# aliabdelkader/FusionTransformer

Measured on AMD Instinct MI355X. Metric: frames/sec fwd+bwd (SemanticKITTI synth), whole job, higher is better.
Workload: dtype f32

## Files before the change

### fusiontransformer_amd/csrc/ftx_attn.hip

```cpp
#include "ftx_common.h"

using namespace ftx;

typedef float f32x16 __attribute__((ext_vector_type(16)));

constexpr int HD = 64;
constexpr int TS = 68;
constexpr float LOG2E = 1.4426950408889634f;
constexpr float LN2 = 0.6931471805599453f;

__device__ inline int acc_row(int g, int h) { return (g & 3) + 8 * (g >> 2) + 4 * h; }

__device__ inline float exp2_raw(float x) { return __builtin_amdgcn_exp2f(x); }

__device__ inline const float *qkv_row(const float *qkv, int b, int t, int which, int hd, int T, int nh) {
  return qkv + ((((int64_t)b * T + t) * 3 + which) * nh + hd) * HD;
}

__device__ inline void load_frag(const float *row, int h, bool valid, float (&f)[32]) {
#pragma unroll
  for (int t = 0; t < 8; ++t) {
    float4 v = make_float4(0.f, 0.f, 0.f, 0.f);
    if (valid) v = *(const float4 *)(row + 8 * t + 4 * h);
    f[4 * t + 0] = v.x; f[4 * t + 1] = v.y; f[4 * t + 2] = v.z; f[4 * t + 3] = v.w;
  }
}

__device__ inline void mfma_lds_x_frag(const float *lds_tile, int l31, int h, const float (&frag)[32], f32x16 &acc) {
  const float *rp = lds_tile + l31 * TS + 4 * h;
#pragma unroll
  for (int t = 0; t < 8; ++t) {
    float4 a = *(const float4 *)(rp + 8 * t);
    acc = __builtin_amdgcn_mfma_f32_32x32x2f32(a.x, frag[4 * t + 0], acc, 0, 0, 0);
    acc = __builtin_amdgcn_mfma_f32_32x32x2f32(a.y, frag[4 * t + 1], acc, 0, 0, 0);
    acc = __builtin_amdgcn_mfma_f32_32x32x2f32(a.z, frag[4 * t + 2], acc, 0, 0, 0);
    acc = __builtin_amdgcn_mfma_f32_32x32x2f32(a.w, frag[4 * t + 3], acc, 0, 0, 0);
  }
}

__device__ inline void mfma_frag_x_lds(const float (&frag)[32], const float *lds_tile, int l31, int h, f32x16 &acc) {
  const float *rp = lds_tile + l31 * TS + 4 * h;
#pragma unroll
  for (int t = 0; t < 8; ++t) {
    float4 b = *(const float4 *)(rp + 8 * t);
    acc = __builtin_amdgcn_mfma_f32_32x32x2f32(frag[4 * t + 0], b.x, acc, 0, 0, 0);
    acc = __builtin_amdgcn_mfma_f32_32x32x2f32(frag[4 * t + 1], b.y, acc, 0, 0, 0);
    acc = __builtin_amdgcn_mfma_f32_32x32x2f32(frag[4 * t + 2], b.z, acc, 0, 0, 0);
    acc = __builtin_amdgcn_mfma_f32_32x32x2f32(frag[4 * t + 3], b.w, acc, 0, 0, 0);
  }
}

__device__ inline void mfma_ldsT_x_acc(const float *lds_tile, int col_off, int l31, int h, const f32x16 &x, f32x16 &out) {
#pragma unroll
  for (int g = 0; g < 16; ++g) {
    float a = lds_tile[acc_row(g, h) * TS + col_off + l31];
    out = __builtin_amdgcn_mfma_f32_32x32x2f32(a, x[g], out, 0, 0, 0);
  }
}

template <int NT>
__device__ inline void tile_prefetch(const float *qkv, int b, int hd, int which, int t0, int T, int nh, int tid, float4 (&r)[512 / NT]) {
#pragma unroll
  for (int q = 0; q < 512 / NT; ++q) {
    int e = q * NT + tid;
    int row = e >> 4, c4 = (e & 15) * 4;
    float4 v = make_float4(0.f, 0.f, 0.f, 0.f);
    if (t0 + row < T) v = *(const float4 *)(qkv_row(qkv, b, t0 + row, which, hd, T, nh) + c4);
    r[q] = v;
  }
}
template <int NT>
__device__ inline void tile_store(float *lds_tile, int tid, const float4 (&r)[512 / NT]) {
#pragma unroll
  for (int q = 0; q < 512 / NT; ++q) {
    int e = q * NT + tid;
    int row = e >> 4, c4 = (e & 15) * 4;
    *(float4 *)&lds_tile[row * TS + c4] = r[q];
  }
}
template <int NT>
__device__ inline void tile_prefetch_o(const float *o, int b, int hd, int t0, int T, int nh, int tid, float4 (&r)[512 / NT]) {
#pragma unroll
  for (int q = 0; q < 512 / NT; ++q) {
    int e = q * NT + tid;
    int row = e >> 4, c4 = (e & 15) * 4;
    float4 v = make_float4(0.f, 0.f, 0.f, 0.f);
    if (t0 + row < T) v = *(const float4 *)(o + (((int64_t)b * T + t0 + row) * nh + hd) * HD + c4);
    r[q] = v;
  }
}

template <int QW>
__device__ inline void group_sync() {
  if (QW == 1) {
    __builtin_amdgcn_fence(__ATOMIC_RELEASE, "wavefront");
    __builtin_amdgcn_wave_barrier();
    __builtin_amdgcn_fence(__ATOMIC_ACQUIRE, "wavefront");
  } else {
    __syncthreads();
  }
}
constexpr int cmax(int a, int b) { return a > b ? a : b; }
template <int QW, int SPLIT, int NREG, int EXTRA>
constexpr int smem_floats() { return cmax(SPLIT * (2 * 32 * TS + EXTRA), cmax(SPLIT / 2, 1) * QW * NREG * 64); }

template <int QW, int SPLIT, int NTILES>
__device__ inline void merge_sum(float *smem, int grp, int wave, int lane, f32x16 (&acc)[NTILES]) {
  if (SPLIT == 1) return;
#pragma unroll
  for (int s = 1; s < SPLIT; s <<= 1) {
    float *cw = smem + ((grp / (2 * s)) * QW + wave) * (16 * NTILES) * 64 + lane;
    __syncthreads();
    if ((grp & (2 * s - 1)) == s) {
#pragma unroll
      for (int t = 0; t < NTILES; ++t)
#pragma unroll
        for (int g = 0; g < 16; ++g) cw[(t * 16 + g) * 64] = acc[t][g];
    }
    __syncthreads();
    if ((grp & (2 * s - 1)) == 0 && grp + s < SPLIT) {
#pragma unroll
      for (int t = 0; t < NTILES; ++t)
#pragma unroll
        for (int g = 0; g < 16; ++g) acc[t][g] += cw[(t * 16 + g) * 64];
    }
  }
}

template <int QW, int SPLIT>
__global__ __launch_bounds__(64 * QW * SPLIT) void attn_fwd_kernel(const float *__restrict__ qkv, int T, int nh, float scale,
                                                                   float *__restrict__ out, float *__restrict__ lse) {
  constexpr int NT = 64 * QW;
  __shared__ __attribute__((aligned(16))) float smem[smem_floats<QW, SPLIT, 34, 0>()];
  const int tid = threadIdx.x % NT, grp = threadIdx.x / NT;
  float *Ks = smem + grp * (2 * 32 * TS), *Vs = Ks + 32 * TS;
  const int wave = tid >> 6, lane = tid & 63, l31 = lane & 31, h = lane >> 5;
  const int hd = blockIdx.y, b = blockIdx.z;
  const int q = blockIdx.x * (32 * QW) + wave * 32 + l31;
  const bool qv = q < T;
  const bool wave_live = blockIdx.x * (32 * QW) + wave * 32 < T;
  const float sl2 = scale * LOG2E;

  float qf[32];
  load_frag(qkv_row(qkv, b, qv ? q : 0, 0, hd, T, nh), h, qv, qf);
#pragma unroll
  for (int i = 0; i < 32; ++i) qf[i] *= sl2;

  f32x16 o0, o1;
#pragma unroll
  for (int g = 0; g < 16; ++g) o0[g] = o1[g] = 0.f;
  float m = -INFINITY, l = 0.f;

  const int ntiles = (T + 31) / 32;
  const int iters = (ntiles + SPLIT - 1) / SPLIT;
  float4 rk[512 / NT], rv[512 / NT];
  tile_prefetch<NT>(qkv, b, hd, 1, grp * 32, T, nh, tid, rk);
  tile_prefetch<NT>(qkv, b, hd, 2, grp * 32, T, nh, tid, rv);
  for (int it = 0; it < iters; ++it) {
    const int kt = it * SPLIT + grp;
    tile_store<NT>(Ks, tid, rk);
    tile_store<NT>(Vs, tid, rv);
    group_sync<QW>();
    if (it + 1 < iters) {
      tile_prefetch<NT>(qkv, b, hd, 1, (kt + SPLIT) * 32, T, nh, tid, rk);
      tile_prefetch<NT>(qkv, b, hd, 2, (kt + SPLIT) * 32, T, nh, tid, rv);
    }
    if (kt < ntiles && wave_live) {
      f32x16 st;
#pragma unroll
      for (int g = 0; g < 16; ++g) st[g] = 0.f;
      mfma_lds_x_frag(Ks, l31, h, qf, st);
      if (kt == ntiles - 1) {
#pragma unroll
        for (int g = 0; g < 16; ++g)
          if (kt * 32 + acc_row(g, h) >= T) st[g] = -INFINITY;
      }
      float mx = fmaxf(fmaxf(fmaxf(st[0], st[1]), fmaxf(st[2], st[3])), fmaxf(fmaxf(st[4], st[5]), fmaxf(st[6], st[7])));
      mx = fmaxf(mx, fmaxf(fmaxf(fmaxf(st[8], st[9]), fmaxf(st[10], st[11])), fmaxf(fmaxf(st[12], st[13]), fmaxf(st[14], st[15]))));
      mx = fmaxf(mx, __shfl_xor(mx, 32, 64));
      const float m_new = fmaxf(m, mx);
      float rs = 0.f;
#pragma unroll
      for (int g = 0; g < 16; ++g) {
        float p = exp2_raw(st[g] - m_new);
        st[g] = p;
        rs += p;
      }
      rs += __shfl_xor(rs, 32, 64);
      if (__any(m_new != m)) {
        const float alpha = exp2_raw(m - m_new);
        l *= alpha;
#pragma unroll
        for (int g = 0; g < 16; ++g) {
          o0[g] *= alpha;
          o1[g] *= alpha;
        }
      }
      l += rs;
      m = m_new;
      mfma_ldsT_x_acc(Vs, 0, l31, h, st, o0);
      mfma_ldsT_x_acc(Vs, 32, l31, h, st, o1);
    }
    group_sync<QW>();
  }
  if (SPLIT > 1) {
#pragma unroll
    for (int s = 1; s < SPLIT; s <<= 1) {
      float *cw = smem + ((grp / (2 * s)) * QW + wave) * 34 * 64 + lane;
      __syncthreads();
      if ((grp & (2 * s - 1)) == s) {
        cw[0] = m;
        cw[64] = l;
#pragma unroll
        for (int g = 0; g < 16; ++g) {
          cw[(2 + g) * 64] = o0[g];
          cw[(18 + g) * 64] = o1[g];
        }
      }
      __syncthreads();
      if ((grp & (2 * s - 1)) == 0 && grp + s < SPLIT) {
        const float m1 = cw[0], l1 = cw[64];
        const float mt = fmaxf(m, m1);
        const float a0 = (m == -INFINITY) ? 0.f : exp2f(m - mt), a1 = (m1 == -INFINITY) ? 0.f : exp2f(m1 - mt);
        l = l * a0 + l1 * a1;
        m = mt;
#pragma unroll
        for (int g = 0; g < 16; ++g) {
          o0[g] = o0[g] * a0 + cw[(2 + g) * 64] * a1;
          o1[g] = o1[g] * a0 + cw[(18 + g) * 64] * a1;
        }
      }
    }
  }
  if (qv && grp == 0) {
    const float inv = 1.f / l;
    float *op = out + (((int64_t)b * T + q) * nh + hd) * HD;
#pragma unroll
    for (int g4 = 0; g4 < 4; ++g4) {
      int r = acc_row(4 * g4, h);
      *(float4 *)(op + r) = make_float4(o0[4 * g4] * inv, o0[4 * g4 + 1] * inv, o0[4 * g4 + 2] * inv, o0[4 * g4 + 3] * inv);
      *(float4 *)(op + 32 + r) = make_float4(o1[4 * g4] * inv, o1[4 * g4 + 1] * inv, o1[4 * g4 + 2] * inv, o1[4 * g4 + 3] * inv);
    }
    if (h == 0) lse[((int64_t)b * nh + hd) * T + q] = (m + log2f(l)) * LN2;
  }
}

__global__ void attn_delta_kernel(const float *__restrict__ o, const float *__restrict__ go, int64_t rows, int T, int nh, float *__restrict__ delta) {
  const int64_t gid = (blockIdx.x * (int64_t)blockDim.x + threadIdx.x) >> 4;
  const int sub = threadIdx.x & 15;
  if (gid >= rows) return;
  float4 a = *(const float4 *)(o + gid * HD + sub * 4);
  float4 g = *(const float4 *)(go + gid * HD + sub * 4);
  float s = a.x * g.x + a.y * g.y + a.z * g.z + a.w * g.w;
#pragma unroll
  for (int off = 8; off > 0; off >>= 1) s += __shfl_xor(s, off, 16);
  if (sub == 0) {
    int64_t bt = gid / nh;
    int hd = (int)(gid - bt * nh);
    int64_t bb = bt / T;
    int t = (int)(bt - bb * T);
    delta[(bb * nh + hd) * T + t] = s;
  }
}

template <int QW, int SPLIT>
__global__ __launch_bounds__(64 * QW * SPLIT) void attn_bwd_kv_kernel(const float *__restrict__ qkv, const float *__restrict__ go,
                                                                      const float *__restrict__ lse, const float *__restrict__ delta, int T,
                                                                      int nh, float scale, float *__restrict__ gqkv) {
  constexpr int NT = 64 * QW;
  __shared__ __attribute__((aligned(16))) float smem[smem_floats<QW, SPLIT, 64, 64>()];
  const int tid = threadIdx.x % NT, grp = threadIdx.x / NT;
  float *Qs = smem + grp * (2 * 32 * TS + 64), *Gs = Qs + 32 * TS, *s_lse = Gs + 32 * TS, *s_delta = s_lse + 32;
  const int wave = tid >> 6, lane = tid & 63, l31 = lane & 31, h = lane >> 5;
  const int hd = blockIdx.y, b = blockIdx.z;
  const int key = blockIdx.x * (32 * QW) + wave * 32 + l31;
  const bool kv = key < T;
  const bool wave_live = blockIdx.x * (32 * QW) + wave * 32 < T;
  const float sl2 = scale * LOG2E;

  float kf[32], vf[32];
  load_frag(qkv_row(qkv, b, kv ? key : 0, 1, hd, T, nh), h, kv, kf);
  load_frag(qkv_row(qkv, b, kv ? key : 0, 2, hd, T, nh), h, kv, vf);
#pragma unroll
  for (int i = 0; i < 32; ++i) kf[i] *= sl2;

  f32x16 acc[4];
#pragma unroll
  for (int t = 0; t < 4; ++t)
#pragma unroll
    for (int g = 0; g < 16; ++g) acc[t][g] = 0.f;

  const int ntiles = (T + 31) / 32;
  const int iters = (ntiles + SPLIT - 1) / SPLIT;
  float4 rq[512 / NT], rg[512 / NT];
  tile_prefetch<NT>(qkv, b, hd, 0, grp * 32, T, nh, tid, rq);
  tile_prefetch_o<NT>(go, b, hd, grp * 32, T, nh, tid, rg);
  for (int it = 0; it < iters; ++it) {
    const int qt = it * SPLIT + grp;
    tile_store<NT>(Qs, tid, rq);
    tile_store<NT>(Gs, tid, rg);
    if (tid < 32) {
      int t = qt * 32 + tid;
      s_lse[tid] = t < T ? lse[((int64_t)b * nh + hd) * T + t] * LOG2E : 0.f;
      s_delta[tid] = t < T ? delta[((int64_t)b * nh + hd) * T + t] : 0.f;
    }
    group_sync<QW>();
    if (it + 1 < iters) {
      tile_prefetch<NT>(qkv, b, hd, 0, (qt + SPLIT) * 32, T, nh, tid, rq);
      tile_prefetch_o<NT>(go, b, hd, (qt + SPLIT) * 32, T, nh, tid, rg);
    }
    if (qt < ntiles && wave_live) {
      f32x16 s, dp;
#pragma unroll
      for (int g = 0; g < 16; ++g) s[g] = dp[g] = 0.f;
      mfma_lds_x_frag(Qs, l31, h, kf, s);
      mfma_lds_x_frag(Gs, l31, h, vf, dp);
#pragma unroll
      for (int g = 0; g < 16; ++g) {
        const int r = acc_row(g, h);
        const float p = exp2_raw(s[g] - s_lse[r]);
        s[g] = p;
        dp[g] = p * (dp[g] - s_delta[r]) * scale;
      }
      if (qt == ntiles - 1) {
#pragma unroll
        for (int g = 0; g < 16; ++g)
          if (qt * 32 + acc_row(g, h) >= T) s[g] = dp[g] = 0.f;
      }
      mfma_ldsT_x_acc(Gs, 0, l31, h, s, acc[0]);
      mfma_ldsT_x_acc(Gs, 32, l31, h, s, acc[1]);
      mfma_ldsT_x_acc(Qs, 0, l31, h, dp, acc[2]);
      mfma_ldsT_x_acc(Qs, 32, l31, h, dp, acc[3]);
    }
    group_sync<QW>();
  }
  merge_sum<QW, SPLIT, 4>(smem, grp, wave, lane, acc);
  if (kv && grp == 0) {
    float *kp = gqkv + ((((int64_t)b * T + key) * 3 + 1) * nh + hd) * HD;
    float *vp = gqkv + ((((int64_t)b * T + key) * 3 + 2) * nh + hd) * HD;
#pragma unroll
    for (int g4 = 0; g4 < 4; ++g4) {
      int r = acc_row(4 * g4, h);
      *(float4 *)(vp + r) = make_float4(acc[0][4 * g4], acc[0][4 * g4 + 1], acc[0][4 * g4 + 2], acc[0][4 * g4 + 3]);
      *(float4 *)(vp + 32 + r) = make_float4(acc[1][4 * g4], acc[1][4 * g4 + 1], acc[1][4 * g4 + 2], acc[1][4 * g4 + 3]);
      *(float4 *)(kp + r) = make_float4(acc[2][4 * g4], acc[2][4 * g4 + 1], acc[2][4 * g4 + 2], acc[2][4 * g4 + 3]);
      *(float4 *)(kp + 32 + r) = make_float4(acc[3][4 * g4], acc[3][4 * g4 + 1], acc[3][4 * g4 + 2], acc[3][4 * g4 + 3]);
    }
  }
}

template <int QW, int SPLIT>
__global__ __launch_bounds__(64 * QW * SPLIT) void attn_bwd_q_kernel(const float *__restrict__ qkv, const float *__restrict__ go,
                                                                     const float *__restrict__ lse, const float *__restrict__ delta, int T,
                                                                     int nh, float scale, float *__restrict__ gqkv) {
  constexpr int NT = 64 * QW;
  __shared__ __attribute__((aligned(16))) float smem[smem_floats<QW, SPLIT, 32, 0>()];
  const int tid = threadIdx.x % NT, grp = threadIdx.x / NT;
  float *Ks = smem + grp * (2 * 32 * TS), *Vs = Ks + 32 * TS;
  const int wave = tid >> 6, lane = tid & 63, l31 = lane & 31, h = lane >> 5;
  const int hd = blockIdx.y, b = blockIdx.z;
  const int q = blockIdx.x * (32 * QW) + wave * 32 + l31;
  const bool qv = q < T;
  const bool wave_live = blockIdx.x * (32 * QW) + wave * 32 < T;
  const float sl2 = scale * LOG2E;

  float qf[32], gf[32];
  load_frag(qkv_row(qkv, b, qv ? q : 0, 0, hd, T, nh), h, qv, qf);
#pragma unroll
  for (int i = 0; i < 32; ++i) qf[i] *= sl2;
  load_frag(go + (((int64_t)b * T + (qv ? q : 0)) * nh + hd) * HD, h, qv, gf);
  const float my_lse = qv ? lse[((int64_t)b * nh + hd) * T + q] * LOG2E : 0.f;
  const float my_delta = qv ? delta[((int64_t)b * nh + hd) * T + q] : 0.f;

  f32x16 acc[2];
#pragma unroll
  for (int g = 0; g < 16; ++g) acc[0][g] = acc[1][g] = 0.f;

  const int ntiles = (T + 31) / 32;
  const int iters = (ntiles + SPLIT - 1) / SPLIT;
  float4 rk[512 / NT], rv[512 / NT];
  tile_prefetch<NT>(qkv, b, hd, 1, grp * 32, T, nh, tid, rk);
  tile_prefetch<NT>(qkv, b, hd, 2, grp * 32, T, nh, tid, rv);
  for (int it = 0; it < iters; ++it) {
    const int kt = it * SPLIT + grp;
    tile_store<NT>(Ks, tid, rk);
    tile_store<NT>(Vs, tid, rv);
    group_sync<QW>();
    if (it + 1 < iters) {
      tile_prefetch<NT>(qkv, b, hd, 1, (kt + SPLIT) * 32, T, nh, tid, rk);
      tile_prefetch<NT>(qkv, b, hd, 2, (kt + SPLIT) * 32, T, nh, tid, rv);
    }
    if (kt < ntiles && wave_live) {
      f32x16 st, dpt;
#pragma unroll
      for (int g = 0; g < 16; ++g) st[g] = dpt[g] = 0.f;
      mfma_lds_x_frag(Ks, l31, h, qf, st);
      mfma_lds_x_frag(Vs, l31, h, gf, dpt);
#pragma unroll
      for (int g = 0; g < 16; ++g) {
        const float p = exp2_raw(st[g] - my_lse);
        dpt[g] = p * (dpt[g] - my_delta) * scale;
      }
      if (kt == ntiles - 1) {
#pragma unroll
        for (int g = 0; g < 16; ++g)
          if (kt * 32 + acc_row(g, h) >= T) dpt[g] = 0.f;
      }
      mfma_ldsT_x_acc(Ks, 0, l31, h, dpt, acc[0]);
      mfma_ldsT_x_acc(Ks, 32, l31, h, dpt, acc[1]);
    }
    group_sync<QW>();
  }
  merge_sum<QW, SPLIT, 2>(smem, grp, wave, lane, acc);
  if (qv && grp == 0) {
    float *qp = gqkv + ((((int64_t)b * T + q) * 3 + 0) * nh + hd) * HD;
#pragma unroll
    for (int g4 = 0; g4 < 4; ++g4) {
      int r = acc_row(4 * g4, h);
      *(float4 *)(qp + r) = make_float4(acc[0][4 * g4], acc[0][4 * g4 + 1], acc[0][4 * g4 + 2], acc[0][4 * g4 + 3]);
      *(float4 *)(qp + 32 + r) = make_float4(acc[1][4 * g4], acc[1][4 * g4 + 1], acc[1][4 * g4 + 2], acc[1][4 * g4 + 3]);
    }
  }
}

static int attn_check(const char *who, int b, int t, int h, int d) {
  FTX_REQUIRE(b >= 1 && t >= 1 && h >= 1, "%s: bad size", who);
  FTX_REQUIRE(d == HD, "%s: head dim must be 64 (got %d)", who, d);
  FTX_REQUIRE(b <= 65535 && h <= 65535, "%s: batch / heads exceed the grid limits", who);
  return FTX_OK;
}

static bool attn_tiling_built(int qw, int split) {
  return (qw == 0 && split == 0) || (qw == 4 && split == 2) || (qw == 2 && (split == 2 || split == 4)) ||
         (qw == 1 && (split == 2 || split == 4 || split == 8));
}
static void attn_config(int b, int t, int h, bool backward, int &qw, int &split) {
  if (qw != 0) return;
  const int64_t wave_tiles = (int64_t)ceil_div(t, 32) * h * b;
  const int64_t simds = 4 * 256;
  if (wave_tiles * 4 <= simds) { qw = 1; split = backward ? 4 : 8; }
  else if (wave_tiles * 2 <= simds) { qw = 2; split = 4; }
  else { qw = 4; split = 2; }
}

#define ATTN_DISPATCH(KERNEL, ...)                                                                               \
  do {                                                                                                           \
    dim3 grid((unsigned)ceil_div(t, 32 * qw), (unsigned)h, (unsigned)b);                                         \
    if (qw == 4) KERNEL<4, 2><<<grid, 512, 0, st>>>(__VA_ARGS__);                                                \
    else if (qw == 2 && split == 2) KERNEL<2, 2><<<grid, 256, 0, st>>>(__VA_ARGS__);                             \
    else if (qw == 2) KERNEL<2, 4><<<grid, 512, 0, st>>>(__VA_ARGS__);                                           \
    else if (split == 2) KERNEL<1, 2><<<grid, 128, 0, st>>>(__VA_ARGS__);                                        \
    else if (split == 4) KERNEL<1, 4><<<grid, 256, 0, st>>>(__VA_ARGS__);                                        \
    else KERNEL<1, 8><<<grid, 512, 0, st>>>(__VA_ARGS__);                                                        \
  } while (0)

extern "C" int ftx_attn_fwd_tiled(const float *qkv, int32_t b, int32_t t, int32_t h, int32_t d, float scale, float *out, float *lse, int32_t qw,
                                  int32_t split, void *stream) {
  int rc = attn_check("ftx_attn_fwd", b, t, h, d);
  if (rc != FTX_OK) return rc;
  FTX_REQUIRE(qkv && out && lse, "ftx_attn_fwd: null pointer");
  FTX_REQUIRE(attn_tiling_built(qw, split), "ftx_attn_fwd_tiled: (%d, %d) is not a built tiling", qw, split);
  hipStream_t st = (hipStream_t)stream;
  attn_config(b, t, h, false, qw, split);
  ATTN_DISPATCH(attn_fwd_kernel, qkv, t, h, scale, out, lse);
  return check_launch("ftx_attn_fwd");
}

extern "C" int ftx_attn_fwd(const float *qkv, int32_t b, int32_t t, int32_t h, int32_t d, float scale, float *out, float *lse, void *stream) {
  return ftx_attn_fwd_tiled(qkv, b, t, h, d, scale, out, lse, 0, 0, stream);
}

extern "C" size_t ftx_attn_bwd_workspace_bytes(int32_t b, int32_t t, int32_t h) {
  if (b <= 0 || t <= 0 || h <= 0) return 256;
  return sizeof(float) * (size_t)b * t * h + 256;
}

extern "C" int ftx_attn_bwd_tiled(const float *qkv, const float *out, const float *grad_out, const float *lse, int32_t b, int32_t t, int32_t h,
                                  int32_t d, float scale, float *grad_qkv, void *workspace, size_t workspace_bytes, int32_t qw, int32_t split,
                                  void *stream) {
  int rc = attn_check("ftx_attn_bwd", b, t, h, d);
  if (rc != FTX_OK) return rc;
  FTX_REQUIRE(qkv && out && grad_out && lse && grad_qkv && workspace, "ftx_attn_bwd: null pointer");
  FTX_REQUIRE(attn_tiling_built(qw, split), "ftx_attn_bwd_tiled: (%d, %d) is not a built tiling", qw, split);
  if (workspace_bytes < ftx_attn_bwd_workspace_bytes(b, t, h)) {
    set_error("ftx_attn_bwd: workspace %zu < required %zu", workspace_bytes, ftx_attn_bwd_workspace_bytes(b, t, h));
    return FTX_EWORKSPACE;
  }
  hipStream_t st = (hipStream_t)stream;
  float *delta = (float *)workspace;
  const int64_t rows = (int64_t)b * t * h;
  attn_delta_kernel<<<(unsigned)ceil_div(rows * 16, 256), 256, 0, st>>>(out, grad_out, rows, t, h, delta);
  attn_config(b, t, h, true, qw, split);
  ATTN_DISPATCH(attn_bwd_kv_kernel, qkv, grad_out, lse, delta, t, h, scale, grad_qkv);
  ATTN_DISPATCH(attn_bwd_q_kernel, qkv, grad_out, lse, delta, t, h, scale, grad_qkv);
  return check_launch("ftx_attn_bwd");
}

extern "C" int ftx_attn_bwd(const float *qkv, const float *out, const float *grad_out, const float *lse, int32_t b, int32_t t, int32_t h,
                            int32_t d, float scale, float *grad_qkv, void *workspace, size_t workspace_bytes, void *stream) {
  return ftx_attn_bwd_tiled(qkv, out, grad_out, lse, b, t, h, d, scale, grad_qkv, workspace, workspace_bytes, 0, 0, stream);
}

typedef __bf16 bf16x8 __attribute__((ext_vector_type(8)));
typedef __bf16 bf16x4 __attribute__((ext_vector_type(4)));

constexpr int RS = 72;
constexpr int CS = 36;
constexpr int IMG = 32 * RS;
static_assert(32 * RS == 64 * CS, "row and col images are the same size");

__device__ inline bf16x4 cvt4(float4 v) { return (bf16x4){(__bf16)v.x, (__bf16)v.y, (__bf16)v.z, (__bf16)v.w}; }

__device__ inline void load_frag_bf16(const float *row, int h, bool valid, bf16x8 (&f)[4]) {
#pragma unroll
  for (int s = 0; s < 4; ++s) {
    float4 a = make_float4(0.f, 0.f, 0.f, 0.f), b = a;
    if (valid) {
      a = *(const float4 *)(row + 16 * s + 8 * h);
      b = *(const float4 *)(row + 16 * s + 8 * h + 4);
    }
    f[s] = __builtin_shufflevector(cvt4(a), cvt4(b), 0, 1, 2, 3, 4, 5, 6, 7);
  }
}
__device__ inline bf16x8 rowimg_frag(const __bf16 *img, int row, int s, int h) { return *(const bf16x8 *)(img + row * RS + 16 * s + 8 * h); }
__device__ inline bf16x8 colimg_frag(const __bf16 *img, int row, int s, int h) {
  const __bf16 *p = img + row * CS + 16 * s + 4 * h;
  return __builtin_shufflevector(*(const bf16x4 *)p, *(const bf16x4 *)(p + 8), 0, 1, 2, 3, 4, 5, 6, 7);
}
__device__ inline bf16x8 acc_frag(const f32x16 &x, int s) {
  bf16x8 r;
#pragma unroll
  for (int j = 0; j < 8; ++j) r[j] = (__bf16)x[8 * s + j];
  return r;
}
__device__ inline f32x16 mfma_bf16(const bf16x8 &a, const bf16x8 &b, const f32x16 &c) {
  return __builtin_amdgcn_mfma_f32_32x32x16_bf16(a, b, c, 0, 0, 0);
}
__device__ inline void mfma_rowimg_x_frag(const __bf16 *img, int l31, int h, const bf16x8 (&frag)[4], f32x16 &acc) {
#pragma unroll
  for (int s = 0; s < 4; ++s) acc = mfma_bf16(rowimg_frag(img, l31, s, h), frag[s], acc);
}
__device__ inline void mfma_colimg_x_acc(const __bf16 *img, int col_off, int l31, int h, const bf16x8 (&x)[2], f32x16 &out) {
#pragma unroll
  for (int s = 0; s < 2; ++s) out = mfma_bf16(colimg_frag(img, col_off + l31, s, h), x[s], out);
}

template <int NT> constexpr int stage_mb() { return (128 + NT - 1) / NT; }
template <int NT>
__device__ inline void tile_prefetch_bf(const float *src, int64_t rstride, int t0, int T, int tid, float4 (&r)[4 * stage_mb<NT>()]) {
#pragma unroll
  for (int q = 0; q < stage_mb<NT>(); ++q) {
    const int e = q * NT + tid, tq = (e >> 4) & 7, c4 = (e & 15) * 4;
#pragma unroll
    for (int i = 0; i < 4; ++i) {
      const int t = t0 + 4 * tq + i;
      float4 v = make_float4(0.f, 0.f, 0.f, 0.f);
      if ((NT <= 128 || e < 128) && t < T) v = *(const float4 *)(src + t * rstride + c4);
      r[4 * q + i] = v;
    }
  }
}
template <int NT>
__device__ inline void tile_store_bf(__bf16 *rowimg, __bf16 *colimg, int tid, const float4 (&r)[4 * stage_mb<NT>()]) {
#pragma unroll
  for (int q = 0; q < stage_mb<NT>(); ++q) {
    const int e = q * NT + tid, tq = e >> 4, c4 = (e & 15) * 4;
    if (NT > 128 && e >= 128) continue;
    if (rowimg) {
#pragma unroll
      for (int i = 0; i < 4; ++i) *(bf16x4 *)(rowimg + (4 * tq + i) * RS + c4) = cvt4(r[4 * q + i]);
    }
    if (colimg) {
      *(bf16x4 *)(colimg + (c4 + 0) * CS + 4 * tq) = (bf16x4){(__bf16)r[4 * q].x, (__bf16)r[4 * q + 1].x, (__bf16)r[4 * q + 2].x, (__bf16)r[4 * q + 3].x};
      *(bf16x4 *)(colimg + (c4 + 1) * CS + 4 * tq) = (bf16x4){(__bf16)r[4 * q].y, (__bf16)r[4 * q + 1].y, (__bf16)r[4 * q + 2].y, (__bf16)r[4 * q + 3].y};
      *(bf16x4 *)(colimg + (c4 + 2) * CS + 4 * tq) = (bf16x4){(__bf16)r[4 * q].z, (__bf16)r[4 * q + 1].z, (__bf16)r[4 * q + 2].z, (__bf16)r[4 * q + 3].z};
      *(bf16x4 *)(colimg + (c4 + 3) * CS + 4 * tq) = (bf16x4){(__bf16)r[4 * q].w, (__bf16)r[4 * q + 1].w, (__bf16)r[4 * q + 2].w, (__bf16)r[4 * q + 3].w};
    }
  }
}
__device__ inline const float *qkv_base(const float *qkv, int b, int which, int hd, int T, int nh) { return qkv_row(qkv, b, 0, which, hd, T, nh); }
template <int QW, int SPLIT, int NREG, int NIMG, int EXTRA>
constexpr int smem_floats_bf16() { return cmax(SPLIT * (NIMG * IMG / 2 + EXTRA), cmax(SPLIT / 2, 1) * QW * NREG * 64); }

template <int QW, int SPLIT>
__global__ __launch_bounds__(64 * QW * SPLIT) void attn_fwd_bf16_kernel(const float *__restrict__ qkv, int T, int nh, float scale,
                                                                        float *__restrict__ out, float *__restrict__ lse) {
  constexpr int NT = 64 * QW;
  __shared__ __attribute__((aligned(16))) float smem[smem_floats_bf16<QW, SPLIT, 34, 2, 0>()];
  const int tid = threadIdx.x % NT, grp = threadIdx.x / NT;
  __bf16 *Ks = (__bf16 *)smem + grp * (2 * IMG), *Vt = Ks + IMG;
  const int wave = tid >> 6, lane = tid & 63, l31 = lane & 31, h = lane >> 5;
  const int hd = blockIdx.y, b = blockIdx.z;
  const int q = blockIdx.x * (32 * QW) + wave * 32 + l31;
  const bool qv = q < T;
  const bool wave_live = blockIdx.x * (32 * QW) + wave * 32 < T;
  const float sl2 = scale * LOG2E;
  const int64_t rstride = 3 * nh * HD;
  const float *kbase = qkv_base(qkv, b, 1, hd, T, nh), *vbase = qkv_base(qkv, b, 2, hd, T, nh);

  bf16x8 qf[4];
  load_frag_bf16(qkv_row(qkv, b, qv ? q : 0, 0, hd, T, nh), h, qv, qf);

  f32x16 o0, o1;
#pragma unroll
  for (int g = 0; g < 16; ++g) o0[g] = o1[g] = 0.f;
  float m = -INFINITY, l = 0.f;

  const int ntiles = (T + 31) / 32;
  const int iters = (ntiles + SPLIT - 1) / SPLIT;
  float4 rk[4 * stage_mb<NT>()], rv[4 * stage_mb<NT>()];
  tile_prefetch_bf<NT>(kbase, rstride, grp * 32, T, tid, rk);
  tile_prefetch_bf<NT>(vbase, rstride, grp * 32, T, tid, rv);
  for (int it = 0; it < iters; ++it) {
    const int kt = it * SPLIT + grp;
    tile_store_bf<NT>(Ks, nullptr, tid, rk);
    tile_store_bf<NT>(nullptr, Vt, tid, rv);
    group_sync<QW>();
    if (it + 1 < iters) {
      tile_prefetch_bf<NT>(kbase, rstride, (kt + SPLIT) * 32, T, tid, rk);
      tile_prefetch_bf<NT>(vbase, rstride, (kt + SPLIT) * 32, T, tid, rv);
    }
    if (kt < ntiles && wave_live) {
      f32x16 st;
#pragma unroll
      for (int g = 0; g < 16; ++g) st[g] = 0.f;
      mfma_rowimg_x_frag(Ks, l31, h, qf, st);
#pragma unroll
      for (int g = 0; g < 16; ++g) st[g] *= sl2;
      if (kt == ntiles - 1) {
#pragma unroll
        for (int g = 0; g < 16; ++g)
          if (kt * 32 + acc_row(g, h) >= T) st[g] = -INFINITY;
      }
      float mx = fmaxf(fmaxf(fmaxf(st[0], st[1]), fmaxf(st[2], st[3])), fmaxf(fmaxf(st[4], st[5]), fmaxf(st[6], st[7])));
      mx = fmaxf(mx, fmaxf(fmaxf(fmaxf(st[8], st[9]), fmaxf(st[10], st[11])), fmaxf(fmaxf(st[12], st[13]), fmaxf(st[14], st[15]))));
      mx = fmaxf(mx, __shfl_xor(mx, 32, 64));
      const float m_new = fmaxf(m, mx);
      float rs = 0.f;
#pragma unroll
      for (int g = 0; g < 16; ++g) {
        float p = exp2_raw(st[g] - m_new);
        st[g] = p;
        rs += p;
      }
      rs += __shfl_xor(rs, 32, 64);
      if (__any(m_new != m)) {
        const float alpha = exp2_raw(m - m_new);
        l *= alpha;
#pragma unroll
        for (int g = 0; g < 16; ++g) {
          o0[g] *= alpha;
          o1[g] *= alpha;
        }
      }
      l += rs;
      m = m_new;
      const bf16x8 pb[2] = {acc_frag(st, 0), acc_frag(st, 1)};
      mfma_colimg_x_acc(Vt, 0, l31, h, pb, o0);
      mfma_colimg_x_acc(Vt, 32, l31, h, pb, o1);
    }
    group_sync<QW>();
  }
  if (SPLIT > 1) {
#pragma unroll
    for (int s = 1; s < SPLIT; s <<= 1) {
      float *cw = smem + ((grp / (2 * s)) * QW + wave) * 34 * 64 + lane;
      __syncthreads();
      if ((grp & (2 * s - 1)) == s) {
        cw[0] = m;
        cw[64] = l;
#pragma unroll
        for (int g = 0; g < 16; ++g) {
          cw[(2 + g) * 64] = o0[g];
          cw[(18 + g) * 64] = o1[g];
        }
      }
      __syncthreads();
      if ((grp & (2 * s - 1)) == 0 && grp + s < SPLIT) {
        const float m1 = cw[0], l1 = cw[64];
        const float mt = fmaxf(m, m1);
        const float a0 = (m == -INFINITY) ? 0.f : exp2f(m - mt), a1 = (m1 == -INFINITY) ? 0.f : exp2f(m1 - mt);
        l = l * a0 + l1 * a1;
        m = mt;
#pragma unroll
        for (int g = 0; g < 16; ++g) {
          o0[g] = o0[g] * a0 + cw[(2 + g) * 64] * a1;
          o1[g] = o1[g] * a0 + cw[(18 + g) * 64] * a1;
        }
      }
    }
  }
  if (qv && grp == 0) {
    const float inv = 1.f / l;
    float *op = out + (((int64_t)b * T + q) * nh + hd) * HD;
#pragma unroll
    for (int g4 = 0; g4 < 4; ++g4) {
      int r = acc_row(4 * g4, h);
      *(float4 *)(op + r) = make_float4(o0[4 * g4] * inv, o0[4 * g4 + 1] * inv, o0[4 * g4 + 2] * inv, o0[4 * g4 + 3] * inv);
      *(float4 *)(op + 32 + r) = make_float4(o1[4 * g4] * inv, o1[4 * g4 + 1] * inv, o1[4 * g4 + 2] * inv, o1[4 * g4 + 3] * inv);
    }
    if (h == 0) lse[((int64_t)b * nh + hd) * T + q] = (m + log2f(l)) * LN2;
  }
}

template <int QW, int SPLIT>
__global__ __launch_bounds__(64 * QW * SPLIT) void attn_bwd_kv_bf16_kernel(const float *__restrict__ qkv, const float *__restrict__ go,
                                                                           const float *__restrict__ lse, const float *__restrict__ delta, int T,
                                                                           int nh, float scale, float *__restrict__ gqkv) {
  constexpr int NT = 64 * QW;
  constexpr int GROUP = 4 * IMG / 2 + 64;
  __shared__ __attribute__((aligned(16))) float smem[smem_floats_bf16<QW, SPLIT, 64, 4, 64>()];
  const int tid = threadIdx.x % NT, grp = threadIdx.x / NT;
  __bf16 *Qs = (__bf16 *)(smem + grp * GROUP), *Qt = Qs + IMG, *Gs = Qt + IMG, *Gt = Gs + IMG;
  float *s_lse = smem + grp * GROUP + 4 * IMG / 2, *s_delta = s_lse + 32;
  const int wave = tid >> 6, lane = tid & 63, l31 = lane & 31, h = lane >> 5;
  const int hd = blockIdx.y, b = blockIdx.z;
  const int key = blockIdx.x * (32 * QW) + wave * 32 + l31;
  const bool kv = key < T;
  const bool wave_live = blockIdx.x * (32 * QW) + wave * 32 < T;
  const float sl2 = scale * LOG2E;
  const float *qbase = qkv_base(qkv, b, 0, hd, T, nh), *gbase = go + ((int64_t)b * T * nh + hd) * HD;

  bf16x8 kf[4], vf[4];
  load_frag_bf16(qkv_row(qkv, b, kv ? key : 0, 1, hd, T, nh), h, kv, kf);
  load_frag_bf16(qkv_row(qkv, b, kv ? key : 0, 2, hd, T, nh), h, kv, vf);

  f32x16 acc[4];
#pragma unroll
  for (int t = 0; t < 4; ++t)
#pragma unroll
    for (int g = 0; g < 16; ++g) acc[t][g] = 0.f;

  const int ntiles = (T + 31) / 32;
  const int iters = (ntiles + SPLIT - 1) / SPLIT;
  float4 rq[4 * stage_mb<NT>()], rg[4 * stage_mb<NT>()];
  tile_prefetch_bf<NT>(qbase, 3 * nh * HD, grp * 32, T, tid, rq);
  tile_prefetch_bf<NT>(gbase, nh * HD, grp * 32, T, tid, rg);
  for (int it = 0; it < iters; ++it) {
    const int qt = it * SPLIT + grp;
    tile_store_bf<NT>(Qs, Qt, tid, rq);
    tile_store_bf<NT>(Gs, Gt, tid, rg);
    if (tid < 32) {
      int t = qt * 32 + tid;
      s_lse[tid] = t < T ? lse[((int64_t)b * nh + hd) * T + t] * LOG2E : 0.f;
      s_delta[tid] = t < T ? delta[((int64_t)b * nh + hd) * T + t] : 0.f;
    }
    group_sync<QW>();
    if (it + 1 < iters) {
      tile_prefetch_bf<NT>(qbase, 3 * nh * HD, (qt + SPLIT) * 32, T, tid, rq);
      tile_prefetch_bf<NT>(gbase, nh * HD, (qt + SPLIT) * 32, T, tid, rg);
    }
    if (qt < ntiles && wave_live) {
      f32x16 s, dp;
#pragma unroll
      for (int g = 0; g < 16; ++g) s[g] = dp[g] = 0.f;
      mfma_rowimg_x_frag(Qs, l31, h, kf, s);
      mfma_rowimg_x_frag(Gs, l31, h, vf, dp);
#pragma unroll
      for (int g = 0; g < 16; ++g) {
        const int r = acc_row(g, h);
        const float p = exp2_raw(s[g] * sl2 - s_lse[r]);
        s[g] = p;
        dp[g] = p * (dp[g] - s_delta[r]) * scale;
      }
      if (qt == ntiles - 1) {
#pragma unroll
        for (int g = 0; g < 16; ++g)
          if (qt * 32 + acc_row(g, h) >= T) s[g] = dp[g] = 0.f;
      }
      const bf16x8 pb[2] = {acc_frag(s, 0), acc_frag(s, 1)}, db[2] = {acc_frag(dp, 0), acc_frag(dp, 1)};
      mfma_colimg_x_acc(Gt, 0, l31, h, pb, acc[0]);
      mfma_colimg_x_acc(Gt, 32, l31, h, pb, acc[1]);
      mfma_colimg_x_acc(Qt, 0, l31, h, db, acc[2]);
      mfma_colimg_x_acc(Qt, 32, l31, h, db, acc[3]);
    }
    group_sync<QW>();
  }
  merge_sum<QW, SPLIT, 4>(smem, grp, wave, lane, acc);
  if (kv && grp == 0) {
    float *kp = gqkv + ((((int64_t)b * T + key) * 3 + 1) * nh + hd) * HD;
    float *vp = gqkv + ((((int64_t)b * T + key) * 3 + 2) * nh + hd) * HD;
#pragma unroll
    for (int g4 = 0; g4 < 4; ++g4) {
      int r = acc_row(4 * g4, h);
      *(float4 *)(vp + r) = make_float4(acc[0][4 * g4], acc[0][4 * g4 + 1], acc[0][4 * g4 + 2], acc[0][4 * g4 + 3]);
      *(float4 *)(vp + 32 + r) = make_float4(acc[1][4 * g4], acc[1][4 * g4 + 1], acc[1][4 * g4 + 2], acc[1][4 * g4 + 3]);
      *(float4 *)(kp + r) = make_float4(acc[2][4 * g4], acc[2][4 * g4 + 1], acc[2][4 * g4 + 2], acc[2][4 * g4 + 3]);
      *(float4 *)(kp + 32 + r) = make_float4(acc[3][4 * g4], acc[3][4 * g4 + 1], acc[3][4 * g4 + 2], acc[3][4 * g4 + 3]);
    }
  }
}

template <int QW, int SPLIT>
__global__ __launch_bounds__(64 * QW * SPLIT) void attn_bwd_q_bf16_kernel(const float *__restrict__ qkv, const float *__restrict__ go,
                                                                          const float *__restrict__ lse, const float *__restrict__ delta, int T,
                                                                          int nh, float scale, float *__restrict__ gqkv) {
  constexpr int NT = 64 * QW;
  __shared__ __attribute__((aligned(16))) float smem[smem_floats_bf16<QW, SPLIT, 32, 3, 0>()];
  const int tid = threadIdx.x % NT, grp = threadIdx.x / NT;
  __bf16 *Ks = (__bf16 *)smem + grp * (3 * IMG), *Kt = Ks + IMG, *Vs = Kt + IMG;
  const int wave = tid >> 6, lane = tid & 63, l31 = lane & 31, h = lane >> 5;
  const int hd = blockIdx.y, b = blockIdx.z;
  const int q = blockIdx.x * (32 * QW) + wave * 32 + l31;
  const bool qv = q < T;
  const bool wave_live = blockIdx.x * (32 * QW) + wave * 32 < T;
  const float sl2 = scale * LOG2E;
  const int64_t rstride = 3 * nh * HD;
  const float *kbase = qkv_base(qkv, b, 1, hd, T, nh), *vbase = qkv_base(qkv, b, 2, hd, T, nh);

  bf16x8 qf[4], gf[4];
  load_frag_bf16(qkv_row(qkv, b, qv ? q : 0, 0, hd, T, nh), h, qv, qf);
  load_frag_bf16(go + (((int64_t)b * T + (qv ? q : 0)) * nh + hd) * HD, h, qv, gf);
  const float my_lse = qv ? lse[((int64_t)b * nh + hd) * T + q] * LOG2E : 0.f;
  const float my_delta = qv ? delta[((int64_t)b * nh + hd) * T + q] : 0.f;

  f32x16 acc[2];
#pragma unroll
  for (int g = 0; g < 16; ++g) acc[0][g] = acc[1][g] = 0.f;

  const int ntiles = (T + 31) / 32;
  const int iters = (ntiles + SPLIT - 1) / SPLIT;
  float4 rk[4 * stage_mb<NT>()], rv[4 * stage_mb<NT>()];
  tile_prefetch_bf<NT>(kbase, rstride, grp * 32, T, tid, rk);
  tile_prefetch_bf<NT>(vbase, rstride, grp * 32, T, tid, rv);
  for (int it = 0; it < iters; ++it) {
    const int kt = it * SPLIT + grp;
    tile_store_bf<NT>(Ks, Kt, tid, rk);
    tile_store_bf<NT>(Vs, nullptr, tid, rv);
    group_sync<QW>();
    if (it + 1 < iters) {
      tile_prefetch_bf<NT>(kbase, rstride, (kt + SPLIT) * 32, T, tid, rk);
      tile_prefetch_bf<NT>(vbase, rstride, (kt + SPLIT) * 32, T, tid, rv);
    }
    if (kt < ntiles && wave_live) {
      f32x16 st, dpt;
#pragma unroll
      for (int g = 0; g < 16; ++g) st[g] = dpt[g] = 0.f;
      mfma_rowimg_x_frag(Ks, l31, h, qf, st);
      mfma_rowimg_x_frag(Vs, l31, h, gf, dpt);
#pragma unroll
      for (int g = 0; g < 16; ++g) {
        const float p = exp2_raw(st[g] * sl2 - my_lse);
        dpt[g] = p * (dpt[g] - my_delta) * scale;
      }
      if (kt == ntiles - 1) {
#pragma unroll
        for (int g = 0; g < 16; ++g)
          if (kt * 32 + acc_row(g, h) >= T) dpt[g] = 0.f;
      }
      const bf16x8 db[2] = {acc_frag(dpt, 0), acc_frag(dpt, 1)};
      mfma_colimg_x_acc(Kt, 0, l31, h, db, acc[0]);
      mfma_colimg_x_acc(Kt, 32, l31, h, db, acc[1]);
    }
    group_sync<QW>();
  }
  merge_sum<QW, SPLIT, 2>(smem, grp, wave, lane, acc);
  if (qv && grp == 0) {
    float *qp = gqkv + ((((int64_t)b * T + q) * 3 + 0) * nh + hd) * HD;
#pragma unroll
    for (int g4 = 0; g4 < 4; ++g4) {
      int r = acc_row(4 * g4, h);
      *(float4 *)(qp + r) = make_float4(acc[0][4 * g4], acc[0][4 * g4 + 1], acc[0][4 * g4 + 2], acc[0][4 * g4 + 3]);
      *(float4 *)(qp + 32 + r) = make_float4(acc[1][4 * g4], acc[1][4 * g4 + 1], acc[1][4 * g4 + 2], acc[1][4 * g4 + 3]);
    }
  }
}

__global__ void attn_delta_bf16_kernel(const float *__restrict__ o, const float *__restrict__ go, int64_t rows, int T, int nh, float *__restrict__ delta) {
  const int64_t gid = (blockIdx.x * (int64_t)blockDim.x + threadIdx.x) >> 4;
  const int sub = threadIdx.x & 15;
  if (gid >= rows) return;
  float4 a = *(const float4 *)(o + gid * HD + sub * 4);
  float4 g = *(const float4 *)(go + gid * HD + sub * 4);
  float s = a.x * (float)(__bf16)g.x + a.y * (float)(__bf16)g.y + a.z * (float)(__bf16)g.z + a.w * (float)(__bf16)g.w;
#pragma unroll
  for (int off = 8; off > 0; off >>= 1) s += __shfl_xor(s, off, 16);
  if (sub == 0) {
    int64_t bt = gid / nh;
    int hd = (int)(gid - bt * nh);
    int64_t bb = bt / T;
    int t = (int)(bt - bb * T);
    delta[(bb * nh + hd) * T + t] = s;
  }
}

static bool attn_bf16_tiling_built(int qw, int split) { return attn_tiling_built(qw, split); }

extern "C" int ftx_attn_fwd_bf16(const float *qkv, int32_t b, int32_t t, int32_t h, int32_t d, float scale, float *out, float *lse, int32_t qw,
                                 int32_t split, void *stream) {
  int rc = attn_check("ftx_attn_fwd_bf16", b, t, h, d);
  if (rc != FTX_OK) return rc;
  FTX_REQUIRE(qkv && out && lse, "ftx_attn_fwd_bf16: null pointer");
  FTX_REQUIRE(attn_bf16_tiling_built(qw, split), "ftx_attn_fwd_bf16: (%d, %d) is not a built tiling", qw, split);
  hipStream_t st = (hipStream_t)stream;
  attn_config(b, t, h, false, qw, split);
  ATTN_DISPATCH(attn_fwd_bf16_kernel, qkv, t, h, scale, out, lse);
  return check_launch("ftx_attn_fwd_bf16");
}

extern "C" int ftx_attn_bwd_bf16(const float *qkv, const float *out, const float *grad_out, const float *lse, int32_t b, int32_t t, int32_t h,
                                 int32_t d, float scale, float *grad_qkv, void *workspace, size_t workspace_bytes, int32_t qw, int32_t split,
                                 void *stream) {
  int rc = attn_check("ftx_attn_bwd_bf16", b, t, h, d);
  if (rc != FTX_OK) return rc;
  FTX_REQUIRE(qkv && out && grad_out && lse && grad_qkv && workspace, "ftx_attn_bwd_bf16: null pointer");
  FTX_REQUIRE(attn_bf16_tiling_built(qw, split), "ftx_attn_bwd_bf16: (%d, %d) is not a built tiling", qw, split);
  if (workspace_bytes < ftx_attn_bwd_workspace_bytes(b, t, h)) {
    set_error("ftx_attn_bwd_bf16: workspace %zu < required %zu", workspace_bytes, ftx_attn_bwd_workspace_bytes(b, t, h));
    return FTX_EWORKSPACE;
  }
  hipStream_t st = (hipStream_t)stream;
  float *delta = (float *)workspace;
  const int64_t rows = (int64_t)b * t * h;
  attn_delta_bf16_kernel<<<(unsigned)ceil_div(rows * 16, 256), 256, 0, st>>>(out, grad_out, rows, t, h, delta);
  attn_config(b, t, h, true, qw, split);
  ATTN_DISPATCH(attn_bwd_kv_bf16_kernel, qkv, grad_out, lse, delta, t, h, scale, grad_qkv);
  ATTN_DISPATCH(attn_bwd_q_bf16_kernel, qkv, grad_out, lse, delta, t, h, scale, grad_qkv);
  return check_launch("ftx_attn_bwd_bf16");
}
```

Measured before the change: 151.0.

## Fuse attention backward dQ into the dK/dV kernel with partial-sum reduction

Merges the separate dQ backward kernel into the dK/dV kernel. Each key block writes its dS tile to shared memory and computes a partial dQ against a transposed K image held in LDS, storing the partial to a workspace buffer. A new reduce kernel then sums the partials across key blocks. This removes the recomputation of S and dP in a second kernel, at the cost of a larger workspace, extra global partial-sum traffic and another launch.

```diff
diff --git a/fusiontransformer_amd/csrc/ftx_attn.hip b/fusiontransformer_amd/csrc/ftx_attn.hip
--- a/fusiontransformer_amd/csrc/ftx_attn.hip
+++ b/fusiontransformer_amd/csrc/ftx_attn.hip
@@ -47,6 +47,18 @@
     acc = __builtin_amdgcn_mfma_f32_32x32x2f32(frag[4 * t + 1], b.y, acc, 0, 0, 0);
     acc = __builtin_amdgcn_mfma_f32_32x32x2f32(frag[4 * t + 2], b.z, acc, 0, 0, 0);
     acc = __builtin_amdgcn_mfma_f32_32x32x2f32(frag[4 * t + 3], b.w, acc, 0, 0, 0);
+  }
+}
+
+__device__ inline void mfma_lds_x_img(const float *lds_tile, const float *img, int stride, int l31, int h, f32x16 &acc) {
+  const float *rp = lds_tile + l31 * TS + 4 * h, *cp = img + 4 * h * stride;
+#pragma unroll
+  for (int t = 0; t < 8; ++t) {
+    float4 a = *(const float4 *)(rp + 8 * t);
+    acc = __builtin_amdgcn_mfma_f32_32x32x2f32(a.x, cp[(8 * t + 0) * stride], acc, 0, 0, 0);
+    acc = __builtin_amdgcn_mfma_f32_32x32x2f32(a.y, cp[(8 * t + 1) * stride], acc, 0, 0, 0);
+    acc = __builtin_amdgcn_mfma_f32_32x32x2f32(a.z, cp[(8 * t + 2) * stride], acc, 0, 0, 0);
+    acc = __builtin_amdgcn_mfma_f32_32x32x2f32(a.w, cp[(8 * t + 3) * stride], acc, 0, 0, 0);
   }
 }
 
@@ -264,23 +276,43 @@
 }
 
 template <int QW, int SPLIT>
-__global__ __launch_bounds__(64 * QW * SPLIT) void attn_bwd_kv_kernel(const float *__restrict__ qkv, const float *__restrict__ go,
-                                                                      const float *__restrict__ lse, const float *__restrict__ delta, int T,
-                                                                      int nh, float scale, float *__restrict__ gqkv) {
+__global__ __launch_bounds__(64 * QW * SPLIT) void attn_bwd_kernel(const float *__restrict__ qkv, const float *__restrict__ go,
+                                                                   const float *__restrict__ lse, const float *__restrict__ delta, int T,
+                                                                   int nh, float scale, float *__restrict__ gqkv, float *__restrict__ dq_part) {
   constexpr int NT = 64 * QW;
-  __shared__ __attribute__((aligned(16))) float smem[smem_floats<QW, SPLIT, 64, 64>()];
+  constexpr int KB = 32 * QW;
+  constexpr int DSS = KB + 4;
+  constexpr int DSF = QW == 1 ? 0 : 32 * DSS;
+  constexpr int GROUP = 2 * 32 * TS + 64 + DSF;
+  static_assert(32 * DSS <= 32 * TS || QW > 1, "the QW = 1 dS image must fit in the dO tile");
+  __shared__ __attribute__((aligned(16))) float smem[cmax(SPLIT * GROUP + 2 * 64 * DSS, cmax(SPLIT / 2, 1) * QW * 64 * 64)];
   const int tid = threadIdx.x % NT, grp = threadIdx.x / NT;
-  float *Qs = smem + grp * (2 * 32 * TS + 64), *Gs = Qs + 32 * TS, *s_lse = Gs + 32 * TS, *s_delta = s_lse + 32;
+  float *Qs = smem + grp * GROUP, *Gs = Qs + 32 * TS, *s_lse = Gs + 32 * TS, *s_delta = s_lse + 32;
+  float *Ds = QW == 1 ? Gs : s_lse + 64;
+  float *Kt = smem + SPLIT * GROUP, *Vt = Kt + 64 * DSS;
   const int wave = tid >> 6, lane = tid & 63, l31 = lane & 31, h = lane >> 5;
   const int hd = blockIdx.y, b = blockIdx.z;
-  const int key = blockIdx.x * (32 * QW) + wave * 32 + l31;
+  const int kb0 = blockIdx.x * KB;
+  const int key = kb0 + wave * 32 + l31;
   const bool kv = key < T;
-  const bool wave_live = blockIdx.x * (32 * QW) + wave * 32 < T;
+  const bool wave_live = kb0 + wave * 32 < T;
+  const bool key_tail = kb0 + KB > T;
   const float sl2 = scale * LOG2E;
 
-  float kf[32], vf[32];
+  for (int e = threadIdx.x; e < 2 * KB * 16; e += NT * SPLIT) {
+    const int which = e / (KB * 16), kk = (e >> 4) % KB, c4 = (e & 15) * 4;
+    float4 v = make_float4(0.f, 0.f, 0.f, 0.f);
+    if (kb0 + kk < T) v = *(const float4 *)(qkv_row(qkv, b, kb0 + kk, 1 + which, hd, T, nh) + c4);
+    float *img = which ? Vt : Kt;
+    img[(c4 + 0) * DSS + kk] = v.x;
+    img[(c4 + 1) * DSS + kk] = v.y;
+    img[(c4 + 2) * DSS + kk] = v.z;
+    img[(c4 + 3) * DSS + kk] = v.w;
+  }
+  __syncthreads();
+
+  float kf[32];
   load_frag(qkv_row(qkv, b, kv ? key : 0, 1, hd, T, nh), h, kv, kf);
-  load_frag(qkv_row(qkv, b, kv ? key : 0, 2, hd, T, nh), h, kv, vf);
 #pragma unroll
   for (int i = 0; i < 32; ++i) kf[i] *= sl2;
 
@@ -292,11 +324,13 @@
 
   const int ntiles = (T + 31) / 32;
   const int iters = (ntiles + SPLIT - 1) / SPLIT;
+  const int64_t part_row0 = (((int64_t)blockIdx.x * gridDim.z + b) * nh + hd) * T;
   float4 rq[512 / NT], rg[512 / NT];
   tile_prefetch<NT>(qkv, b, hd, 0, grp * 32, T, nh, tid, rq);
   tile_prefetch_o<NT>(go, b, hd, grp * 32, T, nh, tid, rg);
   for (int it = 0; it < iters; ++it) {
     const int qt = it * SPLIT + grp;
+    const bool tile_live = qt < ntiles;
     tile_store<NT>(Qs, tid, rq);
     tile_store<NT>(Gs, tid, rg);
     if (tid < 32) {
@@ -309,12 +343,12 @@
       tile_prefetch<NT>(qkv, b, hd, 0, (qt + SPLIT) * 32, T, nh, tid, rq);
       tile_prefetch_o<NT>(go, b, hd, (qt + SPLIT) * 32, T, nh, tid, rg);
     }
-    if (qt < ntiles && wave_live) {
-      f32x16 s, dp;
-#pragma unroll
-      for (int g = 0; g < 16; ++g) s[g] = dp[g] = 0.f;
+    f32x16 s, dp;
+#pragma unroll
+    for (int g = 0; g < 16; ++g) s[g] = dp[g] = 0.f;
+    if (tile_live && wave_live) {
       mfma_lds_x_frag(Qs, l31, h, kf, s);
-      mfma_lds_x_frag(Gs, l31, h, vf, dp);
+      mfma_lds_x_img(Gs, Vt + wave * 32 + l31, DSS, l31, h, dp);
 #pragma unroll
       for (int g = 0; g < 16; ++g) {
         const int r = acc_row(g, h);
@@ -331,6 +365,41 @@
       mfma_ldsT_x_acc(Gs, 32, l31, h, s, acc[1]);
       mfma_ldsT_x_acc(Qs, 0, l31, h, dp, acc[2]);
       mfma_ldsT_x_acc(Qs, 32, l31, h, dp, acc[3]);
+      if (key_tail) {
+#pragma unroll
+        for (int g = 0; g < 16; ++g) dp[g] = kv ? dp[g] : 0.f;
+      }
+    }
+#pragma unroll
+    for (int g = 0; g < 16; ++g) Ds[acc_row(g, h) * DSS + wave * 32 + l31] = dp[g];
+    group_sync<QW>();
+    if (tile_live) {
+      constexpr int NTP = 4 / QW;
+      typedef float f32x4 __attribute__((ext_vector_type(4)));
+      const int r16 = lane & 15, k4 = (lane >> 4) * 4;
+#pragma unroll 1
+      for (int i = 0; i < NTP; ++i) {
+        const int n = wave * NTP + i;
+        f32x4 dq0 = {0.f, 0.f, 0.f, 0.f}, dq1 = dq0;
+        const float *ap = Kt + (16 * n + r16) * DSS + k4, *xp = Ds + r16 * DSS + k4;
+#pragma unroll 4
+        for (int c = 0; c < KB / 16; ++c) {
+          const float4 a = *(const float4 *)(ap + 16 * c);
+          const float4 x0 = *(const float4 *)(xp + 16 * c), x1 = *(const float4 *)(xp + 16 * DSS + 16 * c);
+          dq0 = __builtin_amdgcn_mfma_f32_16x16x4f32(a.x, x0.x, dq0, 0, 0, 0);
+          dq1 = __builtin_amdgcn_mfma_f32_16x16x4f32(a.x, x1.x, dq1, 0, 0, 0);
+          dq0 = __builtin_amdgcn_mfma_f32_16x16x4f32(a.y, x0.y, dq0, 0, 0, 0);
+          dq1 = __builtin_amdgcn_mfma_f32_16x16x4f32(a.y, x1.y, dq1, 0, 0, 0);
+          dq0 = __builtin_amdgcn_mfma_f32_16x16x4f32(a.z, x0.z, dq0, 0, 0, 0);
+          dq1 = __builtin_amdgcn_mfma_f32_16x16x4f32(a.z, x1.z, dq1, 0, 0, 0);
+          dq0 = __builtin_amdgcn_mfma_f32_16x16x4f32(a.w, x0.w, dq0, 0, 0, 0);
+          dq1 = __builtin_amdgcn_mfma_f32_16x16x4f32(a.w, x1.w, dq1, 0, 0, 0);
+        }
+        const int q0 = qt * 32 + r16;
+        float *dst = dq_part + (part_row0 + q0) * HD + 16 * n + k4;
+        if (q0 < T) *(float4 *)dst = make_float4(dq0[0], dq0[1], dq0[2], dq0[3]);
+        if (q0 + 16 < T) *(float4 *)(dst + 16 * HD) = make_float4(dq1[0], dq1[1], dq1[2], dq1[3]);
+      }
     }
     group_sync<QW>();
   }
@@ -349,78 +418,22 @@
   }
 }
 
-template <int QW, int SPLIT>
-__global__ __launch_bounds__(64 * QW * SPLIT) void attn_bwd_q_kernel(const float *__restrict__ qkv, const float *__restrict__ go,
-                                                                     const float *__restrict__ lse, const float *__restrict__ delta, int T,
-                                                                     int nh, float scale, float *__restrict__ gqkv) {
-  constexpr int NT = 64 * QW;
-  __shared__ __attribute__((aligned(16))) float smem[smem_floats<QW, SPLIT, 32, 0>()];
-  const int tid = threadIdx.x % NT, grp = threadIdx.x / NT;
-  float *Ks = smem + grp * (2 * 32 * TS), *Vs = Ks + 32 * TS;
-  const int wave = tid >> 6, lane = tid & 63, l31 = lane & 31, h = lane >> 5;
-  const int hd = blockIdx.y, b = blockIdx.z;
-  const int q = blockIdx.x * (32 * QW) + wave * 32 + l31;
-  const bool qv = q < T;
-  const bool wave_live = blockIdx.x * (32 * QW) + wave * 32 < T;
-  const float sl2 = scale * LOG2E;
-
-  float qf[32], gf[32];
-  load_frag(qkv_row(qkv, b, qv ? q : 0, 0, hd, T, nh), h, qv, qf);
-#pragma unroll
-  for (int i = 0; i < 32; ++i) qf[i] *= sl2;
-  load_frag(go + (((int64_t)b * T + (qv ? q : 0)) * nh + hd) * HD, h, qv, gf);
-  const float my_lse = qv ? lse[((int64_t)b * nh + hd) * T + q] * LOG2E : 0.f;
-  const float my_delta = qv ? delta[((int64_t)b * nh + hd) * T + q] : 0.f;
-
-  f32x16 acc[2];
-#pragma unroll
-  for (int g = 0; g < 16; ++g) acc[0][g] = acc[1][g] = 0.f;
-
-  const int ntiles = (T + 31) / 32;
-  const int iters = (ntiles + SPLIT - 1) / SPLIT;
-  float4 rk[512 / NT], rv[512 / NT];
-  tile_prefetch<NT>(qkv, b, hd, 1, grp * 32, T, nh, tid, rk);
-  tile_prefetch<NT>(qkv, b, hd, 2, grp * 32, T, nh, tid, rv);
-  for (int it = 0; it < iters; ++it) {
-    const int kt = it * SPLIT + grp;
-    tile_store<NT>(Ks, tid, rk);
-    tile_store<NT>(Vs, tid, rv);
-    group_sync<QW>();
-    if (it + 1 < iters) {
-      tile_prefetch<NT>(qkv, b, hd, 1, (kt + SPLIT) * 32, T, nh, tid, rk);
-      tile_prefetch<NT>(qkv, b, hd, 2, (kt + SPLIT) * 32, T, nh, tid, rv);
-    }
-    if (kt < ntiles && wave_live) {
-      f32x16 st, dpt;
-#pragma unroll
-      for (int g = 0; g < 16; ++g) st[g] = dpt[g] = 0.f;
-      mfma_lds_x_frag(Ks, l31, h, qf, st);
-      mfma_lds_x_frag(Vs, l31, h, gf, dpt);
-#pragma unroll
-      for (int g = 0; g < 16; ++g) {
-        const float p = exp2_raw(st[g] - my_lse);
-        dpt[g] = p * (dpt[g] - my_delta) * scale;
-      }
-      if (kt == ntiles - 1) {
-#pragma unroll
-        for (int g = 0; g < 16; ++g)
-          if (kt * 32 + acc_row(g, h) >= T) dpt[g] = 0.f;
-      }
-      mfma_ldsT_x_acc(Ks, 0, l31, h, dpt, acc[0]);
-      mfma_ldsT_x_acc(Ks, 32, l31, h, dpt, acc[1]);
-    }
-    group_sync<QW>();
-  }
-  merge_sum<QW, SPLIT, 2>(smem, grp, wave, lane, acc);
-  if (qv && grp == 0) {
-    float *qp = gqkv + ((((int64_t)b * T + q) * 3 + 0) * nh + hd) * HD;
-#pragma unroll
-    for (int g4 = 0; g4 < 4; ++g4) {
-      int r = acc_row(4 * g4, h);
-      *(float4 *)(qp + r) = make_float4(acc[0][4 * g4], acc[0][4 * g4 + 1], acc[0][4 * g4 + 2], acc[0][4 * g4 + 3]);
-      *(float4 *)(qp + 32 + r) = make_float4(acc[1][4 * g4], acc[1][4 * g4 + 1], acc[1][4 * g4 + 2], acc[1][4 * g4 + 3]);
-    }
-  }
+__global__ void attn_dq_reduce_kernel(const float *__restrict__ part, int nkb, int B, int T, int nh, float *__restrict__ gqkv) {
+  const int64_t i = blockIdx.x * (int64_t)blockDim.x + threadIdx.x;
+  if (i >= (int64_t)B * T * nh * 16) return;
+  const int c = (int)(i & 15) * 4;
+  int64_t r = i >> 4;
+  const int hd = (int)(r % nh);
+  r /= nh;
+  const int t = (int)(r % T), b = (int)(r / T);
+  const int64_t stride = (int64_t)B * nh * T * HD;
+  const float *p = part + (((int64_t)b * nh + hd) * T + t) * HD + c;
+  float4 s = *(const float4 *)p;
+  for (int kb = 1; kb < nkb; ++kb) {
+    const float4 v = *(const float4 *)(p + kb * stride);
+    s.x += v.x; s.y += v.y; s.z += v.z; s.w += v.w;
+  }
+  *(float4 *)(gqkv + (((int64_t)b * T + t) * 3 * nh + hd) * HD + c) = s;
 }
 
 static int attn_check(const char *who, int b, int t, int h, int d) {
@@ -470,9 +483,10 @@
   return ftx_attn_fwd_tiled(qkv, b, t, h, d, scale, out, lse, 0, 0, stream);
 }
 
+static size_t attn_delta_bytes(int32_t b, int32_t t, int32_t h) { return (size_t)ceil_div(sizeof(float) * (size_t)b * t * h, 256) * 256; }
 extern "C" size_t ftx_attn_bwd_workspace_bytes(int32_t b, int32_t t, int32_t h) {
   if (b <= 0 || t <= 0 || h <= 0) return 256;
-  return sizeof(float) * (size_t)b * t * h + 256;
+  return attn_delta_bytes(b, t, h) + sizeof(float) * (size_t)ceil_div(t, 32) * b * h * t * HD;
 }
 
 extern "C" int ftx_attn_bwd_tiled(const float *qkv, const float *out, const float *grad_out, const float *lse, int32_t b, int32_t t, int32_t h,
@@ -491,8 +505,10 @@
   const int64_t rows = (int64_t)b * t * h;
   attn_delta_kernel<<<(unsigned)ceil_div(rows * 16, 256), 256, 0, st>>>(out, grad_out, rows, t, h, delta);
   attn_config(b, t, h, true, qw, split);
-  ATTN_DISPATCH(attn_bwd_kv_kernel, qkv, grad_out, lse, delta, t, h, scale, grad_qkv);
-  ATTN_DISPATCH(attn_bwd_q_kernel, qkv, grad_out, lse, delta, t, h, scale, grad_qkv);
+  float *dq_part = (float *)((char *)workspace + attn_delta_bytes(b, t, h));
+  ATTN_DISPATCH(attn_bwd_kernel, qkv, grad_out, lse, delta, t, h, scale, grad_qkv, dq_part);
+  const int nkb = (int)ceil_div(t, 32 * qw);
+  attn_dq_reduce_kernel<<<(unsigned)ceil_div(rows * 16, 256), 256, 0, st>>>(dq_part, nkb, b, t, h, grad_qkv);
   return check_launch("ftx_attn_bwd");
 }
 
```

After: 152.0, median of 4. About the same (+0.6%).
